# NUSTM/FacialMMT

Measured on AMD Instinct MI355X. Metric: utterances/sec T+A+V forward+bwd, 160-frame face seq, 1/2/4/8 GPU, higher is better.
Workload: dtype bf16; 1 GPU; configs[1]: T+A+V, RoBERTa-large (random init), 160-frame face seq (uint8 112x112 crops, fused pil-bicubic x2 + normalise), batch 4 utterances/GPU, bf16, fwd+bwd+clip+AdamW every step; global_batch=4, parallelism=dp1, hip_graphs=whole step: 2 graphs (fwd+bwd | clip+optimizer), text_encoder_concurrent_with_swin=True, swin_forward_pipelined_across_steps=False, text_encoder_parameters=bf16 with fp32 master weights in the optimizer

## Files before the change

facialmmt_amd/_lib.py:

```python
from __future__ import annotations

import ctypes as C
import os

_HERE = os.path.dirname(os.path.abspath(__file__))
LIB_PATH = os.path.join(_HERE, "libfmmt_hip.so")

F32, BF16 = 0, 1
GENERIC = 0x100
EPI_NONE, EPI_GELU, EPI_GELU_BWD, EPI_GELU_DG, EPI_MUL_AUX = 0, 1, 2, 3, 4
SAVE_DG = 0x200
BATCH_MAJOR = 0x400
RESIZE_PIL, RESIZE_CV2 = 0, 1

_p, _i, _f, _sz, _u64 = C.c_void_p, C.c_int, C.c_float, C.c_size_t, C.c_uint64

SIGNATURES = {
    "fmmt_version": (_i, []),
    "fmmt_linear_fwd": (_i, [_i, _i, _i, _i, _p, _i, _p, _i, _p, _p, _i, _p, _i, _p, _i, _p, _i, _p, _i, _p]),
    "fmmt_linear_splitk_workspace": (_sz, [_i, _i, _i]),
    "fmmt_linear_fwd_splitk": (_i, [_i, _i, _i, _i, _p, _i, _p, _i, _p, _p, _i, _p, _sz, _p]),
    "fmmt_linear_wgrad_workspace": (_sz, [_i, _i, _i, _i]),
    "fmmt_linear_wgrad": (_i, [_i, _i, _i, _i, _p, _i, _p, _i, _p, _p, _p, _i, _i, _p, _sz, _p]),
    "fmmt_linear_wgrad_partials": (_i, [_i, _i, _i, _i, _p, _i, _p, _i, _i, _p, _i, _i, _p, _sz, _p]),
    "fmmt_mlp_fwd": (_i, [_i, _i, _i, _p, _p, _p, _p, _p, _p, _p, _i, _p, _p, _p, _p]),
    "fmmt_mlp_ln_fwd": (_i, [_i, _i, _i, _p, _p, _p, _f, _p, _p, _p, _p, _p, _i, _p, _p, _p, _p, _p, _p, _p]),
    "fmmt_mlp_bwd_input": (_i, [_i, _i, _i, _p, _p, _p, _p, _p, _i, _p, _p, _p]),
    "fmmt_linear_ln_bwd_workspace": (_sz, [_i]),
    "fmmt_linear_ln_bwd": (_i, [_i, _i, _i, _i, _p, _p, _p, _p, _p, _p, _p, _p, _p, _p, _p, _sz, _p]),
    "fmmt_mlp_ln_bwd_input_workspace": (_sz, [_i]),
    "fmmt_mlp_ln_bwd_input": (_i, [_i, _i, _i, _p, _p, _p, _p, _p, _i, _p, _p, _p, _p, _p, _p, _p, _p, _p, _sz, _p]),
    "fmmt_linear_wgrad_finish": (_i, [_i, _i, _i, _i, _p, _p, _p, _sz, _p]),
    "fmmt_layernorm_fwd": (_i, [_i, _i, _i, _p, _p, _p, _f, _p, _p, _p, _i, _p]),
    "fmmt_layernorm_bwd_workspace": (_sz, [_i]),
    "fmmt_layernorm_bwd": (_i, [_i, _i, _i, _p, _p, _p, _p, _p, _p, _p, _p, _p, _i, _p, _sz, _p]),
    "fmmt_window_attn_fwd": (_i, [_i, _i, _i, _i, _i, _i, _i, _p, _p, _p, _p, _i, _i, _f, _p, _p, _p]),
    "fmmt_window_attn_bwd_workspace": (_sz, [_i]),
    "fmmt_window_attn_bwd": (_i, [_i, _i, _i, _i, _i, _i, _i, _p, _p, _p, _p, _p, _p, _p, _i, _i, _f, _p, _p, _p, _sz, _p]),
    "fmmt_window_block_fwd": (_i, [_i, _i, _i, _i, _i, _i, _i, _p, _p, _p, _f, _p, _p, _p, _p, _p, _p, _f, _p, _p, _p, _p, _p, _p, _p, _p]),
    "fmmt_window_block_fwd_ref": (_i, [_i, _i, _i, _i, _i, _i, _i, _p, _p, _p, _f, _p, _p, _p, _p, _p, _p, _f, _p, _p, _p, _p, _p, _p, _p, _p]),
    "fmmt_window_block_attn_bwd": (_i, [_i, _i, _i, _i, _i, _i, _i, _p, _p, _p, _p, _p, _p, _p, _p, _p, _f, _p, _p, _p, _p, _sz, _p]),
    "fmmt_window_block_attn_bwd_ref": (_i, [_i, _i, _i, _i, _i, _i, _i, _p, _p, _p, _p, _p, _p, _p, _p, _p, _f, _p, _p, _p, _p, _sz, _p]),
    "fmmt_linear_fwd_seg3": (_i, [_i, _i, _i, _i, _p, _i, _p, _p, _p, _i, _i, _p, _p, _p, _p, _i, _p]),
    "fmmt_select_frames_fwd": (_i, [_i, _i, _i, _i, _i, _i, _p, _p, _p, _p, _f, _p, _p, _p, _p]),
    "fmmt_select_frames_bwd": (_i, [_i, _i, _i, _i, _i, _i, _p, _p, _p, _p]),
    "fmmt_mha_fwd": (_i, [_i, _i, _i, _i, _i, _i, _p, _i, _p, _p, _i, _f, _p, _f, _u64, _p, _p, _i, _p, _p]),
    "fmmt_mha_bwd": (_i, [_i, _i, _i, _i, _i, _i, _p, _i, _p, _p, _i, _f, _p, _f, _u64, _p, _p, _p, _i, _p, _p, _i, _p, _p, _i, _p]),
    "fmmt_mha_avg_weights": (_i, [_i, _i, _i, _i, _i, _i, _p, _i, _p, _i, _f, _p, _f, _u64, _p, _p, _p, _p]),
    "fmmt_patch_im2col": (_i, [_i, _i, _p, _p, _p]),
    "fmmt_patch_col2im": (_i, [_i, _i, _p, _p, _p]),
    "fmmt_batchnorm1d_fwd": (_i, [_i, _i, _i, _p, _p, _p, _p, _p, _f, _f, _i, _p, _p, _p, _p]),
    "fmmt_batchnorm1d_bwd": (_i, [_i, _i, _i, _p, _p, _p, _p, _p, _i, _p, _p, _p, _p]),
    "fmmt_posemb_scale_fwd": (_i, [_i, _i, _i, _i, _p, _p, _f, _p, _p]),
    "fmmt_scale": (_i, [_i, _sz, _p, _f, _p, _p]),
    "fmmt_colsum": (_i, [_i, _i, _i, _i, _p, _i, _p, _p]),
    "fmmt_cast_batch": (_i, [_i, _i, _p, _p]),
    "fmmt_layernorm_bwd_bf16_workspace": (_sz, [_i, _i]),
    "fmmt_layernorm_bwd_bf16": (_i, [_i, _i, _f, _p, _p, _p, _p, _p, _p, _p, _sz, _p]),
    "fmmt_dropadd_ln_fwd": (_i, [_i, _i, _i, _f, _p, _p, _p, _p, _f, _u64, _p, _u64, _p, _p, _p]),
    "fmmt_dropadd_ln_bwd_workspace": (_sz, [_i, _i]),
    "fmmt_dropadd_ln_bwd": (_i, [_i, _i, _i, _f, _p, _p, _p, _f, _u64, _p, _u64, _p, _p, _p, _p, _p, _p, _sz, _p]),
    "fmmt_plm_dropadd_ln_fwd": (_i, [_i, _i, _f, _p, _p, _p, _p, _f, _u64, _p, _u64, _p, _p, _p]),
    "fmmt_embedding_bwd": (_i, [_i, _i, _i, _p, C.c_int64, _p, _p, _p]),
    "fmmt_plm_gelu_bwd_colsum_workspace": (_sz, [_i, _i]),
    "fmmt_plm_gelu_bwd_colsum": (_i, [_i, _i, _p, _p, _p, _p, _p, _sz, _p]),
    "fmmt_plm_dropadd_ln_bwd_workspace": (_sz, [_i, _i]),
    "fmmt_plm_dropadd_ln_bwd": (_i, [_i, _i, _f, _p, _p, _p, _f, _u64, _p, _u64, _p, _p, _p, _p, _p, _p, _sz, _p]),
    "fmmt_grad_handover": (_i, [_i, _i, _p, _p, _p, _p]),
    "fmmt_adamw_batch": (_i, [_i, _i, _p, _p, _p, _p, _f, _f, _f, _f, _f, _i, _p]),
    "fmmt_resize_table": (_i, [_i, _i, _i, _p, _p]),
    "fmmt_resize_band_rows": (_i, [_p, _i]),
    "fmmt_patch_embed_u8": (_i, [_i, _i, _i, _i, _p, _p, _p, _p, _p]),
    "fmmt_patch_embed_ln_fwd": (_i, [_i, _i, _i, _i, _p, _p, _p, _p, _p, _f, _p, _p, _p, _p, _p]),
    "fmmt_patch_embed_u8_ln_fwd": (_i, [_i, _i, _i, _i, _p, _p, _p, _p, _p, _p, _p, _f, _p, _p, _p, _p, _p, _p]),
    "fmmt_emotion_head_fwd": (_i, [_i, _i, _i, _i, _i, _p, _i, _p, _p, _p, _p, _p, _f, _p, _p, _p]),
    "fmmt_eval_accumulate": (_i, [_i, _i, _i, _p, _i, _p, _p, _p, _p, _p, _p, C.c_int64, C.c_int64, _p]),
}

FMMT_EINVAL, FMMT_EALIGN, FMMT_EWORKSPACE = -1, -2, -3
_ERR = {-1: "FMMT_EINVAL (bad shape / unsupported size)", -2: "FMMT_EALIGN (pointer or leading dimension not 16-byte aligned)",
        -3: "FMMT_EWORKSPACE (workspace too small)"}

_lib = None


class FmmtError(RuntimeError):
    pass


def load():
    global _lib
    if _lib is not None:
        return _lib
    if not os.path.exists(LIB_PATH):
# ... 25 lines not shown
```

facialmmt_amd/build.py:

```python
from __future__ import annotations

import glob
import os
import subprocess
import sys
from concurrent.futures import ThreadPoolExecutor

HERE = os.path.dirname(os.path.abspath(__file__))
CSRC = os.path.join(HERE, "csrc")
OUT = os.path.join(HERE, "libfmmt_hip.so")
SOURCES = ["gemm.hip", "layernorm.hip", "attn.hip", "wattn_mfma.hip", "wattn_bwd_ref.hip", "wblock.hip", "wblock_ref.hip", "mha_mfma.hip", "misc.hip", "preproc.hip", "mlp_fused.hip", "mlp_ref.hip", "patch_ln.hip", "lin_lnbwd.hip", "plm_fused.hip", "frame_filter.hip", "eval.hip"]
FLAGS = ["--offload-arch=gfx950", "-O3", "-std=c++17", "-fPIC", "-ffp-contract=fast"]


def _stale(target, deps):
    if not os.path.exists(target):
        return True
    t = os.path.getmtime(target)
    return any(os.path.getmtime(d) > t for d in deps)


def build(force: bool = False, verbose: bool = True, tag: str = "") -> str:
    hipcc = os.environ.get("HIPCC", "/opt/rocm/bin/hipcc")
    tag = tag or os.environ.get("FMMT_BUILD_TAG", "")
    csrc = os.environ.get("FMMT_CSRC_DIR", CSRC) if tag else CSRC
    headers = sorted(glob.glob(os.path.join(csrc, "*.h"))) + [os.path.join(csrc, "..", "..", "include", "fmmt.h")]
    objdir = os.path.join(HERE, "build_" + tag if tag else "build")
    out = os.path.join(HERE, f"libfmmt_hip_{tag}.so") if tag else OUT
    os.makedirs(objdir, exist_ok=True)
    jobs = []
    for s in SOURCES:
        src = os.path.join(csrc, s)
        obj = os.path.join(objdir, s.replace(".hip", ".o"))
        if force or _stale(obj, [src] + headers):
            jobs.append((src, obj))

    def cc(job):
        src, obj = job
        cmd = [hipcc] + FLAGS + os.environ.get("FMMT_CFLAGS", "").split() + ["-c", src, "-o", obj]
        if verbose:
            print(" ".join(cmd), flush=True)
        subprocess.run(cmd, check=True)

    with ThreadPoolExecutor(max_workers=4) as ex:
        list(ex.map(cc, jobs))
    objs = [os.path.join(objdir, s.replace(".hip", ".o")) for s in SOURCES]
    if force or jobs or _stale(out, objs):
        cmd = [hipcc, "--offload-arch=gfx950", "-shared", "-fPIC", "-o", out] + objs
        if verbose:
            print(" ".join(cmd), flush=True)
        subprocess.run(cmd, check=True)
    return out


if __name__ == "__main__":
    print(build(force="--force" in sys.argv))
```

facialmmt_amd/csrc/attn.hip:

```cpp
#include "fmmt_common.h"
#include "../../include/fmmt.h"
#include "wattn_args.h"
#include "mha_args.h"
#include <stdlib.h>

namespace {

constexpr int TOK = 49;
constexpr int WS = 7;
constexpr int HD = 32;
constexpr int KP = 36;
constexpr int BP = 50;
constexpr int WA_BWD_WAVES_PER_HEAD_MAX = 256;


template <typename T> __device__ __forceinline__ void load_row32(const T* p, float* r) {
    constexpr int VEC = Vec<T>::N;
#pragma unroll
    for (int c = 0; c < HD / VEC; ++c) {
        const Vec<T> v = ldvec<T>(p + c * VEC);
#pragma unroll
        for (int e = 0; e < VEC; ++e) r[c * VEC + e] = v.get(e);
    }
}
// ... 490 lines not shown
#pragma unroll 2
        for (int ii = 0; ii < MT; ++ii) {
            if (i0 + ii >= p.Lq) break;
            const float pij = __expf(ldot<D>(Qs + ii * P, kreg) + kb - Ls[ii]);
            const float ks = keep_scale(p, bh, i0 + ii, j);
            if constexpr (WHICH == 0) {
                laxpy<D>(acc, pij * ks, Gs + ii * P);
            } else {
                const float dP = ldot<D>(Gs + ii * P, vreg) * ks;
                laxpy<D>(acc, pij * (dP - Dl[ii]), Qs + ii * P);
            }
        }
    }
    if (active) {
        T* dst = reinterpret_cast<T*>(WHICH == 0 ? p.dv : p.dk);
        store_row<T, D>(dst + p.rk(j, b) * p.lddkv + h * D, acc);
    }
}

int mha_check(int dtype, int Lq, int Lk, int B, int E, int nH) {
    if (dtype != FMMT_BF16 && dtype != FMMT_F32) return FMMT_EINVAL;
    if (Lq <= 0 || Lk <= 0 || B <= 0 || nH <= 0 || E % nH) return FMMT_EINVAL;
    const int hd = E / nH;
    if (hd != 64 && hd != 32) return FMMT_EINVAL;
    return 0;
}


template <typename T>
__global__ __launch_bounds__(128) void mha_avg_weights_kernel(MhaArgs p, float* __restrict__ w) {
    extern __shared__ float qs[];
    const int i = blockIdx.x, b = blockIdx.y, hd = p.E / p.nH;
    const T* qg = reinterpret_cast<const T*>(p.q) + p.rq(i, b) * p.ldq;
    const T* kg = reinterpret_cast<const T*>(p.k);
    for (int c = threadIdx.x; c < p.E; c += 128) qs[c] = to_f32(qg[c]) * p.scale;
    __syncthreads();
    for (int j = threadIdx.x; j < p.Lk; j += 128) {
        const T* kr = kg + p.rk(j, b) * p.ldkv;
        const float kb = key_bias(p, b, j);
        float acc = 0.f;
        for (int h = 0; h < p.nH; ++h) {
            const int bh = b * p.nH + h;
            float s = 0.f;
            for (int d = 0; d < hd; ++d) s += qs[h * hd + d] * to_f32(kr[h * hd + d]);
            acc += __expf(s + kb - p.lse[(size_t)bh * p.Lq + i]) * keep_scale(p, bh, i, j);
        }
        w[((size_t)b * p.Lq + i) * p.Lk + j] = acc / (float)p.nH;
    }
}

}

extern "C" int fmmt_window_attn_fwd(int dtype, int n_img, int H, int W, int C, int num_heads, int shift,
                                    const void* qkv, const float* table, const int32_t* index,
                                    const float* mask, int nW_mask, int mask_is_shift, float scale,
                                    void* out, float* lse, void* stream) {
    if (int e = wa_check(dtype, n_img, H, W, C, num_heads, shift)) return e;
    if (mask && nW_mask <= 0) return FMMT_EINVAL;
    WaArgs a{};
    a.n_img = n_img; a.H = H; a.W = W; a.C = C; a.nH = num_heads; a.shift = shift; a.qkv = qkv; a.table = table;
    a.index = index; a.mask = mask; a.nW_mask = nW_mask; a.mask_is_shift = mask_is_shift; a.scale = scale; a.out = out; a.lse = lse;
    const int B_ = n_img * (H / WS) * (W / WS);
    a.groups_per_head = wa_groups_per_head(B_, num_heads, false, dtype == FMMT_BF16);
    a.xcd_grouped = wa_xcd_grouped(a.groups_per_head, dtype == FMMT_BF16);
    hipStream_t st = reinterpret_cast<hipStream_t>(stream);
    dim3 grid(num_heads * a.groups_per_head);
    if (dtype == FMMT_BF16) return fmmt_wattn_mfma_fwd_launch(a, (int)grid.x, st);
    hipLaunchKernelGGL(wattn_fwd_kernel<float>, grid, dim3(256), 0, st, a);
    FMMT_CHECK_LAUNCH();
    return 0;
}

static size_t wa_part_bytes(int num_heads) { return ((size_t)num_heads * (WA_BWD_WAVES_PER_HEAD_MAX + 1) * TOK * TOK * sizeof(float) + 255) / 256 * 256; }

extern "C" size_t fmmt_window_attn_bwd_workspace(int num_heads) {
    return wa_part_bytes(num_heads) + WA_SINK_BYTES;
}

extern "C" int fmmt_window_attn_bwd(int dtype, int n_img, int H, int W, int C, int num_heads, int shift,
                                    const void* qkv, const void* out, const void* dout, const float* lse,
                                    const float* table, const int32_t* index, const float* mask, int nW_mask,
                                    int mask_is_shift, float scale, void* dqkv, float* dtable,
                                    void* workspace, size_t workspace_bytes, void* stream) {
    const bool want_generic = (dtype & FMMT_GENERIC) != 0;
    dtype &= 0xff;
    if (int e = wa_check(dtype, n_img, H, W, C, num_heads, shift)) return e;
    if (mask && nW_mask <= 0) return FMMT_EINVAL;
    if (workspace_bytes < fmmt_window_attn_bwd_workspace(num_heads)) return FMMT_EWORKSPACE;
    const bool generic_ok = !mask || (mask_is_shift && shift > 0);
    if (want_generic && !generic_ok) return FMMT_EINVAL;
    const bool generic = want_generic || (dtype == FMMT_F32 && generic_ok);
    WaArgs a{};
    a.n_img = n_img; a.H = H; a.W = W; a.C = C; a.nH = num_heads; a.shift = shift; a.qkv = qkv; a.table = table;
    a.index = index; a.mask = mask; a.nW_mask = nW_mask; a.mask_is_shift = mask_is_shift; a.scale = scale; a.out = const_cast<void*>(out);
    a.lse = const_cast<float*>(lse); a.dout = dout; a.dqkv = dqkv; a.part = reinterpret_cast<float*>(workspace);
    a.sink = reinterpret_cast<char*>(workspace) + wa_part_bytes(num_heads);
    const int B_ = n_img * (H / WS) * (W / WS);
    a.groups_per_head = wa_groups_per_head(B_, num_heads, true, dtype == FMMT_BF16);
    a.xcd_grouped = wa_xcd_grouped(a.groups_per_head, dtype == FMMT_BF16);
    hipStream_t st = reinterpret_cast<hipStream_t>(stream);
    if (generic) {
        a.groups_per_head = fmmt_wattn_bwd_groups(B_, num_heads, 1);
        a.xcd_grouped = 0;
        if (int rc = fmmt_wattn_bwd_ref_launch(dtype, a, num_heads * a.groups_per_head, st)) return rc;
        return fmmt_wattn_dtable_finish(a.part, num_heads, a.groups_per_head, index, dtable, st);
    }
    dim3 grid(num_heads * a.groups_per_head);
    if (dtype == FMMT_BF16) {
        if (int rc = fmmt_wattn_mfma_bwd_launch(a, (int)grid.x, st)) return rc;
    } else {
        hipLaunchKernelGGL(wattn_bwd_kernel<float>, grid, dim3(256), 0, st, a);
        FMMT_CHECK_LAUNCH();
    }
    return fmmt_wattn_dtable_finish(a.part, num_heads, dtype == FMMT_BF16 ? a.groups_per_head : a.groups_per_head * 4, index, dtable, st);
}

static int wba_run(bool generic, int dtype, int n_img, int H, int W, int C, int num_heads, int shift,
                   const void* xn, const void* dy, const void* attn_out, const float* lse,
                   const void* wqkv, const float* bqkv, const void* wproj,
                   const float* table, const int32_t* index, float scale, const float* rowscale,
                   void* dqkv, float* dtable, void* workspace, size_t workspace_bytes, void* stream) {
    if (int e = wa_check(dtype, n_img, H, W, C, num_heads, shift)) return e;
    generic = generic || dtype == FMMT_F32;
    if ((dtype != FMMT_BF16 && dtype != FMMT_F32) || (C != 96 && C != 192) || (generic && C != 96)) return FMMT_EINVAL;
    if (!xn || !dy || !attn_out || !lse || !wqkv || !wproj || !table || !index || !dqkv || !dtable || !workspace) return FMMT_EINVAL;
    if (workspace_bytes < fmmt_window_attn_bwd_workspace(num_heads)) return FMMT_EWORKSPACE;
    WaArgs a{};
    a.n_img = n_img; a.H = H; a.W = W; a.C = C; a.nH = num_heads; a.shift = shift; a.table = table; a.index = index; a.scale = scale;
    a.mask_is_shift = shift > 0; a.out = const_cast<void*>(attn_out); a.lse = const_cast<float*>(lse); a.dout = dy; a.dqkv = dqkv;
    a.part = reinterpret_cast<float*>(workspace);
    a.sink = reinterpret_cast<char*>(workspace) + wa_part_bytes(num_heads);
    a.xn = xn; a.wqkv = wqkv; a.bqkv = bqkv; a.wproj = wproj; a.rowscale = rowscale;
    const int B_ = n_img * (H / WS) * (W / WS);
    hipStream_t st = reinterpret_cast<hipStream_t>(stream);
    if (generic) {
        a.groups_per_head = fmmt_wattn_bwd_groups(B_, num_heads, 1);
        if (int rc = fmmt_wattn_bwd_ref_launch(dtype, a, num_heads * a.groups_per_head, st)) return rc;
        return fmmt_wattn_dtable_finish(a.part, num_heads, a.groups_per_head, index, dtable, st);
    }
    a.groups_per_head = fmmt_wattn_bwd_groups(B_, num_heads, 4);
    a.xcd_grouped = wa_xcd_grouped(a.groups_per_head, true);
    if (int rc = fmmt_wattn_mfma_bwd_rc_launch(a, num_heads * a.groups_per_head, st)) return rc;
    return fmmt_wattn_dtable_finish(a.part, num_heads, a.groups_per_head, index, dtable, st);
}

extern "C" int fmmt_window_block_attn_bwd(int dtype, int n_img, int H, int W, int C, int num_heads, int shift,
                                          const void* xn, const void* dy, const void* attn_out, const float* lse,
                                          const void* wqkv, const float* bqkv, const void* wproj,
                                          const float* table, const int32_t* index, float scale, const float* rowscale,
                                          void* dqkv, float* dtable, void* workspace, size_t workspace_bytes, void* stream) {
    return wba_run(false, dtype, n_img, H, W, C, num_heads, shift, xn, dy, attn_out, lse, wqkv, bqkv, wproj, table, index, scale, rowscale,
                   dqkv, dtable, workspace, workspace_bytes, stream);
}

extern "C" int fmmt_window_block_attn_bwd_ref(int dtype, int n_img, int H, int W, int C, int num_heads, int shift,
                                              const void* xn, const void* dy, const void* attn_out, const float* lse,
                                              const void* wqkv, const float* bqkv, const void* wproj,
                                              const float* table, const int32_t* index, float scale, const float* rowscale,
                                              void* dqkv, float* dtable, void* workspace, size_t workspace_bytes, void* stream) {
    return wba_run(true, dtype, n_img, H, W, C, num_heads, shift, xn, dy, attn_out, lse, wqkv, bqkv, wproj, table, index, scale, rowscale,
                   dqkv, dtable, workspace, workspace_bytes, stream);
}

int fmmt_wattn_dtable_finish(float* part, int num_heads, int parts_per_head, const int32_t* index, float* dtable, hipStream_t st) {
    const int nt = (2 * WS - 1) * (2 * WS - 1) * num_heads;
    float* dense = part + (size_t)num_heads * WA_BWD_WAVES_PER_HEAD_MAX * TOK * TOK;
    const int nd = num_heads * TOK * TOK;
    hipLaunchKernelGGL(wattn_dense_kernel, dim3((nd + 63) / 64), dim3(256), 0, st, part, num_heads, parts_per_head, dense);
    FMMT_CHECK_LAUNCH();
    hipLaunchKernelGGL(wattn_dtable_kernel, dim3(nt), dim3(64), 0, st, dense, index, num_heads, dtable);
    FMMT_CHECK_LAUNCH();
    return 0;
}

int fmmt_wattn_bwd_groups(int B_, int num_heads, int windows_per_iteration) {
    int g = 256 / num_heads;
    const int maxg = (B_ + windows_per_iteration - 1) / windows_per_iteration;
    if (g > maxg) g = maxg;
    if (g > WA_BWD_WAVES_PER_HEAD_MAX) g = WA_BWD_WAVES_PER_HEAD_MAX;
    if (g >= 8) g &= ~7;
    return g < 1 ? 1 : g;
}

#define FMMT_MHA_DISPATCH(KERNEL, GRIDX)                                                             \
    do {                                                                                             \
        dim3 grid((GRIDX), B * num_heads);                                                           \
        const int hd = E / num_heads;                                                                \
        if (dtype == FMMT_BF16) {                                                                    \
// ... 67 lines not shown
```

facialmmt_amd/csrc/wattn_args.h:

```cpp
#pragma once
#include <hip/hip_runtime.h>
#include <stdint.h>

struct WaArgs {
    int n_img, H, W, C, nH, shift;
    const void* qkv;
    const float* table;
    const int32_t* index;
    const float* mask;
    int nW_mask;
    int mask_is_shift;
    float scale;
    void* out;
    float* lse;
    const void* dout;
    void* dqkv;
    float* part;
    int groups_per_head;
    int xcd_grouped;
    const void* xn;
    const void* wqkv;
    const float* bqkv;
    const void* wproj;
    const float* rowscale;
    void* sink;
};
constexpr size_t WA_SINK_BYTES = 16 * 1024;

int fmmt_wattn_mfma_fwd_launch(const WaArgs& a, int grid, hipStream_t st);
int fmmt_wattn_mfma_bwd_launch(const WaArgs& a, int grid, hipStream_t st);
int fmmt_wattn_mfma_bwd_rc_launch(const WaArgs& a, int grid, hipStream_t st);
int fmmt_wattn_bwd_ref_launch(int dtype, const WaArgs& a, int grid, hipStream_t st);

int fmmt_wattn_dtable_finish(float* part, int num_heads, int parts_per_head, const int32_t* index, float* dtable, hipStream_t st);
int fmmt_wattn_bwd_groups(int B_, int num_heads, int windows_per_iteration);
```

include/fmmt.h:

```cpp
#ifndef FMMT_H
#define FMMT_H
#include <stddef.h>
#include <stdint.h>

#ifdef __cplusplus
extern "C" {
#endif

#define FMMT_F32 0
#define FMMT_BF16 1
#define FMMT_GENERIC 0x100
#define FMMT_SAVE_DG 0x200
#define FMMT_BATCH_MAJOR 0x400

#define FMMT_EINVAL (-1)
#define FMMT_EALIGN (-2)
#define FMMT_EWORKSPACE (-3)

#define FMMT_EPI_GELU 1
#define FMMT_EPI_GELU_BWD 2
#define FMMT_EPI_GELU_DG 3
#define FMMT_EPI_MUL_AUX 4

int fmmt_version(void);

int fmmt_linear_fwd(int dtype, int M, int N, int K,
                    const void* x, int ldx, const void* w, int ldw, const float* bias,
                    void* y, int ldy, void* y_pre,
                    int epi, const void* aux, int ldaux,
                    const void* res, int ldres, const float* rowscale, int rows_per_scale,
                    void* stream);

int fmmt_linear_fwd_seg3(int dtype, int M, int N, int K, const void* x, int ldx, const void* w0, const void* w1, const void* w2, int ldw,
                         int seg_mode, const float* bias0, const float* bias1, const float* bias2, void* y, int ldy, void* stream);

size_t fmmt_linear_splitk_workspace(int M, int N, int K);
int fmmt_linear_fwd_splitk(int dtype, int M, int N, int K, const void* x, int ldx, const void* w, int ldw,
                           const float* bias, void* y, int ldy, void* workspace, size_t workspace_bytes,
                           void* stream);

size_t fmmt_linear_wgrad_workspace(int dtype, int M, int N, int K);
int fmmt_linear_wgrad(int dtype, int M, int N, int K,
                      const void* dy, int lddy, const void* x, int ldx,
                      float* dw, float* db, const float* rowscale, int rows_per_scale, int x_epi,
                      void* workspace, size_t workspace_bytes, void* stream);
int fmmt_linear_wgrad_partials(int dtype, int M, int N, int K,
                               const void* dy, int lddy, const void* x, int ldx, int want_bias,
                               const float* rowscale, int rows_per_scale, int x_epi,
                               void* workspace, size_t workspace_bytes, void* stream);
int fmmt_linear_wgrad_finish(int dtype, int M, int N, int K, float* dw, float* db,
                             const void* workspace, size_t workspace_bytes, void* stream);

int fmmt_mlp_fwd(int dtype, int M, int C, const void* x, const void* w1, const float* b1, const void* w2, const float* b2,
                 const void* res, const float* rowscale, int rows_per_scale, void* y, void* h_pre, void* h_act, void* stream);

int fmmt_mlp_ln_fwd(int dtype, int M, int C, const void* x, const float* ln_gamma, const float* ln_beta, float eps,
                    const void* w1, const float* b1, const void* w2, const float* b2, const float* rowscale, int rows_per_scale,
                    void* y, void* xn, float* mean, float* rstd, void* h_pre, void* h_act, void* stream);

int fmmt_mlp_bwd_input(int dtype, int M, int C, const void* dy, const void* h_pre, const void* w2t, const void* w1t,
                       const float* rowscale, int rows_per_scale, void* dh, void* dx, void* stream);

size_t fmmt_mlp_ln_bwd_input_workspace(int C);
int fmmt_mlp_ln_bwd_input(int dtype, int M, int C, const void* dy, const void* h_pre, const void* w2t, const void* w1t,
                          const float* rowscale, int rows_per_scale, const void* x, const float* mean, const float* rstd,
                          const float* ln_gamma, void* dh, void* dx, float* dgamma, float* dbeta, void* workspace,
                          size_t workspace_bytes, void* stream);

int fmmt_layernorm_fwd(int dtype, int M, int C, const void* x, const float* gamma, const float* beta,
                       float eps, void* y, float* mean, float* rstd, int merge_hw, void* stream);

size_t fmmt_layernorm_bwd_workspace(int C);
int fmmt_layernorm_bwd(int dtype, int M, int C, const void* dy, const void* x, const float* mean,
                       const float* rstd, const float* gamma, const void* add, void* dx,
                       float* dgamma, float* dbeta, int merge_hw,
                       void* workspace, size_t workspace_bytes, void* stream);

int fmmt_window_attn_fwd(int dtype, int n_img, int H, int W, int C, int num_heads, int shift,
                         const void* qkv, const float* table, const int32_t* index,
                         const float* mask, int nW_mask, int mask_is_shift, float scale,
                         void* out, float* lse, void* stream);

size_t fmmt_window_attn_bwd_workspace(int num_heads);
int fmmt_window_attn_bwd(int dtype, int n_img, int H, int W, int C, int num_heads, int shift,
                         const void* qkv, const void* out, const void* dout, const float* lse,
                         const float* table, const int32_t* index, const float* mask, int nW_mask,
                         int mask_is_shift, float scale, void* dqkv, float* dtable,
                         void* workspace, size_t workspace_bytes, void* stream);

int fmmt_window_block_fwd(int dtype, int n_img, int H, int W, int C, int num_heads, int shift,
                          const void* x, const float* ln_gamma, const float* ln_beta, float eps,
                          const void* wqkv, const float* bqkv, const void* wproj, const float* bproj,
                          const float* table, const int32_t* index, float scale, const float* rowscale,
                          void* y, void* xn, void* attn_out, float* mean, float* rstd, float* lse, void* stream);
int fmmt_window_block_fwd_ref(int dtype, int n_img, int H, int W, int C, int num_heads, int shift,
                              const void* x, const float* ln_gamma, const float* ln_beta, float eps,
// ... 109 lines not shown
```

Before: 74.11 utterances/s.

## Add 16-wave single-workgroup-per-CU window attention backward kernel

Adds a new bf16 window-attention backward kernel that runs 1024-thread workgroups. Each workgroup holds eight windows' K/Q/dO/V tiles in LDS with a swizzled layout and reads them back with transposed LDS loads. It computes dQ, dK, dV and the relative-position-bias gradient, and reduces d(bias) across waves in shared memory. It is enabled by default for C==768 and for shifted C==192 layers, with environment and flag overrides to force the old path. The aim is higher occupancy and more work per CU than the existing MFMA backward kernel. The cost is a large LDS footprint per workgroup and a serial cross-wave bias reduction.

```diff
diff --git a/facialmmt_amd/_lib.py b/facialmmt_amd/_lib.py
--- a/facialmmt_amd/_lib.py
+++ b/facialmmt_amd/_lib.py
@@ -10,6 +10,8 @@
 GENERIC = 0x100
 EPI_NONE, EPI_GELU, EPI_GELU_BWD, EPI_GELU_DG, EPI_MUL_AUX = 0, 1, 2, 3, 4
 SAVE_DG = 0x200
+WATTN_OCC = 0x1000
+WATTN_OLD = 0x800
 BATCH_MAJOR = 0x400
 RESIZE_PIL, RESIZE_CV2 = 0, 1
 
diff --git a/facialmmt_amd/build.py b/facialmmt_amd/build.py
--- a/facialmmt_amd/build.py
+++ b/facialmmt_amd/build.py
@@ -9,7 +9,7 @@
 HERE = os.path.dirname(os.path.abspath(__file__))
 CSRC = os.path.join(HERE, "csrc")
 OUT = os.path.join(HERE, "libfmmt_hip.so")
-SOURCES = ["gemm.hip", "layernorm.hip", "attn.hip", "wattn_mfma.hip", "wattn_bwd_ref.hip", "wblock.hip", "wblock_ref.hip", "mha_mfma.hip", "misc.hip", "preproc.hip", "mlp_fused.hip", "mlp_ref.hip", "patch_ln.hip", "lin_lnbwd.hip", "plm_fused.hip", "frame_filter.hip", "eval.hip"]
+SOURCES = ["gemm.hip", "layernorm.hip", "attn.hip", "wattn_mfma.hip", "wattn_bwd_occ.hip", "wattn_bwd_ref.hip", "wblock.hip", "wblock_ref.hip", "mha_mfma.hip", "misc.hip", "preproc.hip", "mlp_fused.hip", "mlp_ref.hip", "patch_ln.hip", "lin_lnbwd.hip", "plm_fused.hip", "frame_filter.hip", "eval.hip"]
 FLAGS = ["--offload-arch=gfx950", "-O3", "-std=c++17", "-fPIC", "-ffp-contract=fast"]
 
 
diff --git a/facialmmt_amd/csrc/attn.hip b/facialmmt_amd/csrc/attn.hip
--- a/facialmmt_amd/csrc/attn.hip
+++ b/facialmmt_amd/csrc/attn.hip
@@ -596,7 +596,7 @@
                                     const float* table, const int32_t* index, const float* mask, int nW_mask,
                                     int mask_is_shift, float scale, void* dqkv, float* dtable,
                                     void* workspace, size_t workspace_bytes, void* stream) {
-    const bool want_generic = (dtype & FMMT_GENERIC) != 0;
+    const bool want_generic = (dtype & FMMT_GENERIC) != 0, want_old = (dtype & FMMT_WATTN_OLD) != 0, want_occ = (dtype & FMMT_WATTN_OCC) != 0;
     dtype &= 0xff;
     if (int e = wa_check(dtype, n_img, H, W, C, num_heads, shift)) return e;
     if (mask && nW_mask <= 0) return FMMT_EINVAL;
@@ -618,6 +618,18 @@
         a.xcd_grouped = 0;
         if (int rc = fmmt_wattn_bwd_ref_launch(dtype, a, num_heads * a.groups_per_head, st)) return rc;
         return fmmt_wattn_dtable_finish(a.part, num_heads, a.groups_per_head, index, dtable, st);
+    }
+#ifndef FMMT_WATTN_OCC_DEFAULT
+#define FMMT_WATTN_OCC_DEFAULT 1
+#endif
+    static const int occ_on = fmmt_const("FMMT_WATTN_OCC", FMMT_WATTN_OCC_DEFAULT);
+    const bool occ_won = C == 768 || (C == 192 && mask && mask_is_shift);
+    if (dtype == FMMT_BF16 && !want_old && (want_occ || (occ_on && occ_won))) {
+        if (const int g = fmmt_wattn_bwd_occ_groups(a, B_, WA_BWD_WAVES_PER_HEAD_MAX)) {
+            a.groups_per_head = g;
+            if (int rc = fmmt_wattn_bwd_occ_launch(a, WA_BWD_WAVES_PER_HEAD_MAX, st)) return rc;
+            return fmmt_wattn_dtable_finish(a.part, num_heads, g, index, dtable, st);
+        }
     }
     dim3 grid(num_heads * a.groups_per_head);
     if (dtype == FMMT_BF16) {
diff --git a/facialmmt_amd/csrc/wattn_args.h b/facialmmt_amd/csrc/wattn_args.h
--- a/facialmmt_amd/csrc/wattn_args.h
+++ b/facialmmt_amd/csrc/wattn_args.h
@@ -30,6 +30,8 @@
 int fmmt_wattn_mfma_fwd_launch(const WaArgs& a, int grid, hipStream_t st);
 int fmmt_wattn_mfma_bwd_launch(const WaArgs& a, int grid, hipStream_t st);
 int fmmt_wattn_mfma_bwd_rc_launch(const WaArgs& a, int grid, hipStream_t st);
+int fmmt_wattn_bwd_occ_groups(const WaArgs& a, int B_, int max_groups);
+int fmmt_wattn_bwd_occ_launch(const WaArgs& a, int part_groups_max, hipStream_t st);
 int fmmt_wattn_bwd_ref_launch(int dtype, const WaArgs& a, int grid, hipStream_t st);
 
 int fmmt_wattn_dtable_finish(float* part, int num_heads, int parts_per_head, const int32_t* index, float* dtable, hipStream_t st);
diff --git a/facialmmt_amd/csrc/wattn_bwd_occ.hip b/facialmmt_amd/csrc/wattn_bwd_occ.hip
--- /dev/null
+++ b/facialmmt_amd/csrc/wattn_bwd_occ.hip
@@ -0,0 +1,323 @@
+#include "fmmt_common.h"
+#include "../../include/fmmt.h"
+#include "wattn_args.h"
+#include "wattn_geom.h"
+
+namespace {
+
+constexpr float OCC_LOG2E = 1.4426950408889634f;
+constexpr int OCC_NP = 8, OCC_NT = OCC_NP * 128;
+constexpr int OCC_TILE = 64 * HD;
+constexpr int OCC_TILES_B = 4 * OCC_NP * OCC_TILE * 2, OCC_STATS_B = 2 * OCC_NP * 64 * 4, OCC_BIAS_B = TOK * BPM * 4;
+constexpr int OCC_LDS = OCC_TILES_B + OCC_STATS_B + OCC_BIAS_B;
+static_assert(OCC_LDS <= 160 * 1024, "one workgroup per CU");
+static_assert((size_t)OCC_NT * 16 <= WA_SINK_BYTES, "every thread owns 16 bytes of the store sink");
+static_assert(3 * OCC_TILE * 2 >= TOK * TOK * 4, "the d(bias) reduction tile lies over the first three K tiles");
+
+__device__ __forceinline__ int occ_chunk(int c, int rq) { return c ^ ((4 - rq) & 3); }
+
+__device__ __forceinline__ int occ_row_off(int t, int li, int lg) { return (t * 16 + li) * HD + occ_chunk(lg, (li >> 2) & 3) * 8; }
+
+__device__ __forceinline__ bf16x8 occ_tr_frag(const bf16* tile, int rb, int lg, int dt, int li) {
+    const bf16* a0 = tile + (32 * rb + 4 * lg + (li >> 2)) * HD + occ_chunk(li & 3, lg) * 8 + dt * 4;
+    union { struct { s16x4 lo, hi; } s; bf16x8 v; } u;
+    u.s.lo = __builtin_amdgcn_ds_read_tr16_b64_v4i16((lds_s16x4*)(a0));
+    u.s.hi = __builtin_amdgcn_ds_read_tr16_b64_v4i16((lds_s16x4*)(a0 + 16 * HD));
+    return u.v;
+}
+
+struct OccSlot { int di, dj; bool valid; };
+__device__ __forceinline__ OccSlot occ_slot_of(int slot) {
+    OccSlot S;
+    S.valid = slot < TOK;
+    const int cs = S.valid ? slot : TOK - 1;
+    S.di = cs / WS;
+    S.dj = cs - S.di * WS;
+    return S;
+}
+
+template <int MM>
+__global__ __launch_bounds__(OCC_NT) void wattn_bwd_occ_kernel(WaArgs p) {
+    __shared__ __attribute__((aligned(16))) char smem_occ[OCC_LDS];
+    bf16* const tiles = reinterpret_cast<bf16*>(smem_occ);
+    float (*Ls)[64] = reinterpret_cast<float (*)[64]>(smem_occ + OCC_TILES_B);
+    float (*Dl)[64] = Ls + OCC_NP;
+    float* Bs = reinterpret_cast<float*>(smem_occ + OCC_TILES_B + OCC_STATS_B);
+    const int lane = threadIdx.x & 63, wave = __builtin_amdgcn_readfirstlane(threadIdx.x >> 6);
+    const int pair = wave >> 1, h = wave & 1;
+    const int li = lane & 15, lg = lane >> 4;
+#define OCC_LANE() int l_ = lane; asm volatile("" : "+v"(l_)); const int li = l_ & 15, lg = l_ >> 4
+
+    int head, grp;
+    {
+        const int b = blockIdx.x, gph = p.groups_per_head;
+        if (p.xcd_grouped) {
+            const int u = (b >> 4) * 8 + (b & 7);
+            if (u >= (p.nH >> 1) * gph) return;
+            const int hp = u / gph;
+            head = hp * 2 + ((b >> 3) & 1);
+            grp = u - hp * gph;
+        } else {
+            head = b / gph;
+            grp = b - head * gph;
+        }
+    }
+    const int nW = (p.H / WS) * (p.W / WS), B_ = p.n_img * nW;
+    const int stride = p.groups_per_head * OCC_NP;
+    const bf16* __restrict__ qkv = reinterpret_cast<const bf16*>(p.qkv);
+    const bf16* __restrict__ og = reinterpret_cast<const bf16*>(p.out);
+    const bf16* __restrict__ dog = reinterpret_cast<const bf16*>(p.dout);
+    bf16* __restrict__ dqkv = reinterpret_cast<bf16*>(p.dqkv);
+    const LaneGeom G = lane_geom(li, lg, p.shift);
+    bf16 *kt_ = tiles + pair * OCC_TILE, *qt_ = kt_ + OCC_NP * OCC_TILE, *gt_ = qt_ + OCC_NP * OCC_TILE, *vt_ = gt_ + OCC_NP * OCC_TILE;
+    bf16* const sink_w = reinterpret_cast<bf16*>(p.sink) + wave * 64 * 8;
+
+    for (int t = threadIdx.x; t < TOK * BPM; t += OCC_NT) {
+        const int q = t / BPM, k = t - q * BPM;
+        Bs[t] = k < TOK ? p.table[p.index[q * TOK + k] * p.nH + head] * OCC_LOG2E : NEG_BIG;
+    }
+    const float sc2 = p.scale * OCC_LOG2E;
+    f32x4 dbias[2][4];
+#pragma unroll
+    for (int a = 0; a < 2; ++a)
+#pragma unroll
+        for (int b = 0; b < 4; ++b) dbias[a][b] = f32x4{0.f, 0.f, 0.f, 0.f};
+
+    const int iters = (B_ + stride - 1) / stride;
+    for (int it = 0; it < iters; ++it) {
+        const int b_raw = it * stride + grp * OCC_NP + pair;
+        const bool wactive = b_raw < B_;
+        const int b_ = wactive ? b_raw : B_ - 1;
+        const WinPos P = win_pos(p, b_);
+        int tok[2];
+        bf16x8 qf[2], kf[2], gf[2], vv[2], of[2];
+        float ls[2], dl[2];
+        {
+        OCC_LANE();
+#pragma unroll
+        for (int a = 0; a < 2; ++a) {
+            const OccSlot own = occ_slot_of((2 * h + a) * 16 + li);
+            tok[a] = (int)tok_of(p, P, own.di, own.dj);
+            const bf16* row = qkv + (size_t)tok[a] * 3 * p.C + head * HD + lg * 8;
+            qf[a] = ld_frag(row);
+            kf[a] = ld_frag(row + p.C);
+            vv[a] = ld_frag(row + 2 * p.C);
+            gf[a] = ld_frag(dog + (size_t)tok[a] * p.C + head * HD + lg * 8);
+            of[a] = ld_frag(og + (size_t)tok[a] * p.C + head * HD + lg * 8);
+            const int slot = (2 * h + a) * 16 + li;
+            ls[a] = p.lse[((size_t)b_ * p.nH + head) * TOK + (slot < TOK ? slot : TOK - 1)];
+        }
+        }
+        __syncthreads();
+        {
+        OCC_LANE();
+#pragma unroll
+        for (int a = 0; a < 2; ++a) {
+            const int slot = (2 * h + a) * 16 + li;
+            const bool valid = slot < TOK;
+            float d = 0.f;
+#pragma unroll
+            for (int e = 0; e < 8; ++e) d += (float)gf[a][e] * (float)of[a][e];
+            dl[a] = xor_sum(d);
+            ls[a] = valid ? ls[a] * OCC_LOG2E : 1.0e30f;
+            const int off = occ_row_off(2 * h + a, li, lg);
+            kf[a] = valid ? kf[a] : zero_frag();
+            qf[a] = valid ? qf[a] : zero_frag();
+            gf[a] = valid ? gf[a] : zero_frag();
+            vv[a] = valid ? vv[a] : zero_frag();
+            *reinterpret_cast<bf16x8*>(kt_ + off) = kf[a];
+            *reinterpret_cast<bf16x8*>(qt_ + off) = qf[a];
+            *reinterpret_cast<bf16x8*>(gt_ + off) = gf[a];
+            *reinterpret_cast<bf16x8*>(vt_ + off) = vv[a];
+            if (lg == 0) {
+                Ls[pair][slot] = ls[a];
+                Dl[pair][slot] = dl[a];
+            }
+        }
+        }
+        __syncthreads();
+
+#pragma unroll
+        for (int a = 0; a < 2; ++a) {
+            OCC_LANE();
+            const int qt = 2 * h + a;
+            const int q = qt * 16 + li;
+            const float* brow = Bs + (q < TOK ? q : TOK - 1) * BPM + lg * 4;
+            float ds[8];
+            bf16x8 dpk[2];
+            const unsigned mb = (MM == 1) ? std_mask_bits(G, P, qt) : 0u;
+            const bf16x8 qfa = ld_frag(qt_ + occ_row_off(qt, li, lg)), gfa = ld_frag(gt_ + occ_row_off(qt, li, lg));
+            const float lsa = Ls[pair][q], dla = Dl[pair][q];
+#pragma unroll
+            for (int ktp = 0; ktp < 4; ++ktp) {
+                const int kt = ktp;
+                const bf16x8 kfk = ld_frag(kt_ + occ_row_off(kt, li, lg));
+                const f32x4 sa = __builtin_amdgcn_mfma_f32_16x16x32_bf16(kfk, qfa, f32x4{0.f, 0.f, 0.f, 0.f}, 0, 0, 0);
+                const bf16x8 vfk = ld_frag(vt_ + occ_row_off(kt, li, lg));
+                const f32x4 dp = __builtin_amdgcn_mfma_f32_16x16x32_bf16(vfk, gfa, f32x4{0.f, 0.f, 0.f, 0.f}, 0, 0, 0);
+                const f32x4 b = *reinterpret_cast<const f32x4*>(brow + kt * 16);
+                const unsigned mbk = mb >> (kt * 4);
+#pragma unroll
+                for (int r = 0; r < 4; ++r) {
+                    const float s = sa[r] * sc2 + b[r];
+                    float pij = __builtin_amdgcn_exp2f(s - lsa);
+                    if constexpr (MM == 1) pij = ((mbk >> r) & 1u) ? 0.0f : pij;
+                    const float d = pij * (dp[r] - dla);
+                    ds[(ktp & 1) * 4 + r] = d;
+                    if (wactive) dbias[a][ktp][r] += d;
+                }
+                if (ktp & 1) {
+                    dpk[ktp >> 1] = pack8(&ds[0], &ds[4]);
+                    __builtin_amdgcn_sched_barrier(0);
+                }
+            }
+            const bf16x8 d0 = dpk[0], d1 = dpk[1];
+            __builtin_amdgcn_sched_barrier(0);
+            bf16x8 kT[2][2];
+#pragma unroll
+            for (int ks = 0; ks < 2; ++ks)
+#pragma unroll
+                for (int dt = 0; dt < 2; ++dt) kT[ks][dt] = occ_tr_frag(kt_, ks, lg, dt, li);
+            f32x4 a0 = {0.f, 0.f, 0.f, 0.f}, a1 = {0.f, 0.f, 0.f, 0.f};
+            a0 = __builtin_amdgcn_mfma_f32_16x16x32_bf16(kT[0][0], d0, a0, 0, 0, 0);
+            a0 = __builtin_amdgcn_mfma_f32_16x16x32_bf16(kT[1][0], d1, a0, 0, 0, 0);
+            a1 = __builtin_amdgcn_mfma_f32_16x16x32_bf16(kT[0][1], d0, a1, 0, 0, 0);
+            a1 = __builtin_amdgcn_mfma_f32_16x16x32_bf16(kT[1][1], d1, a1, 0, 0, 0);
+            {
+                bf16x8 ob;
+#pragma unroll
+                for (int r = 0; r < 4; ++r) { ob[r] = (bf16)(a0[r] * p.scale); ob[4 + r] = (bf16)(a1[r] * p.scale); }
+                *reinterpret_cast<bf16x8*>((wactive && q < TOK) ? dqkv + (size_t)tok[a] * 3 * p.C + head * HD + lg * 8 : sink_w + l_ * 8) = ob;
+            }
+            __builtin_amdgcn_sched_barrier(0);
+        }
+
+#pragma unroll
+        for (int a = 0; a < 2; ++a) {
+            OCC_LANE();
+            const int kt = 2 * h + a;
+            const int key = kt * 16 + li;
+            float pp[8], ds[8];
+            bf16x8 ppk[2], dpk[2];
+            const unsigned mb = (MM == 1) ? std_mask_bits(G, P, kt) : 0u;
+            const bf16x8 kfa = ld_frag(kt_ + occ_row_off(kt, li, lg)), vfa = ld_frag(vt_ + occ_row_off(kt, li, lg));
+            const float* bcol = Bs + key;
+#pragma unroll
+            for (int qtp = 0; qtp < 4; ++qtp) {
+                const int qt = qtp;
+                const bf16x8 qfq = ld_frag(qt_ + occ_row_off(qt, li, lg));
+                const bf16x8 gfq = ld_frag(gt_ + occ_row_off(qt, li, lg));
+                const f32x4 sa = __builtin_amdgcn_mfma_f32_16x16x32_bf16(qfq, kfa, f32x4{0.f, 0.f, 0.f, 0.f}, 0, 0, 0);
+                const f32x4 dp = __builtin_amdgcn_mfma_f32_16x16x32_bf16(gfq, vfa, f32x4{0.f, 0.f, 0.f, 0.f}, 0, 0, 0);
+                const f32x4 lq = *reinterpret_cast<const f32x4*>(&Ls[pair][qt * 16 + lg * 4]);
+                const f32x4 dq = *reinterpret_cast<const f32x4*>(&Dl[pair][qt * 16 + lg * 4]);
+                const unsigned mbq = mb >> (qt * 4);
+#pragma unroll
+                for (int r = 0; r < 4; ++r) {
+                    const int q = qt * 16 + lg * 4 + r;
+                    const float s = sa[r] * sc2 + bcol[(q < TOK ? q : TOK - 1) * BPM];
+                    float pij = __builtin_amdgcn_exp2f(s - lq[r]);
+                    if constexpr (MM == 1) pij = ((mbq >> r) & 1u) ? 0.0f : pij;
+                    pp[(qtp & 1) * 4 + r] = pij;
+                    ds[(qtp & 1) * 4 + r] = pij * (dp[r] - dq[r]);
+                }
+                if (qtp & 1) {
+                    ppk[qtp >> 1] = pack8(&pp[0], &pp[4]);
+                    dpk[qtp >> 1] = pack8(&ds[0], &ds[4]);
+                }
+                __builtin_amdgcn_sched_barrier(0);
+            }
+            const bf16x8 p0 = ppk[0], p1 = ppk[1], d0 = dpk[0], d1 = dpk[1];
+            __builtin_amdgcn_sched_barrier(0);
+            f32x4 v0 = {0.f, 0.f, 0.f, 0.f}, v1 = {0.f, 0.f, 0.f, 0.f}, k0 = {0.f, 0.f, 0.f, 0.f}, k1 = {0.f, 0.f, 0.f, 0.f};
+            {
+                bf16x8 gT[2][2];
+#pragma unroll
+                for (int qs = 0; qs < 2; ++qs)
+#pragma unroll
+                    for (int dt = 0; dt < 2; ++dt) gT[qs][dt] = occ_tr_frag(gt_, qs, lg, dt, li);
+                v0 = __builtin_amdgcn_mfma_f32_16x16x32_bf16(gT[0][0], p0, v0, 0, 0, 0);
+                v0 = __builtin_amdgcn_mfma_f32_16x16x32_bf16(gT[1][0], p1, v0, 0, 0, 0);
+                v1 = __builtin_amdgcn_mfma_f32_16x16x32_bf16(gT[0][1], p0, v1, 0, 0, 0);
+                v1 = __builtin_amdgcn_mfma_f32_16x16x32_bf16(gT[1][1], p1, v1, 0, 0, 0);
+            }
+            {
+                bf16x8 qT[2][2];
+#pragma unroll
+                for (int qs = 0; qs < 2; ++qs)
+#pragma unroll
+                    for (int dt = 0; dt < 2; ++dt) qT[qs][dt] = occ_tr_frag(qt_, qs, lg, dt, li);
+                k0 = __builtin_amdgcn_mfma_f32_16x16x32_bf16(qT[0][0], d0, k0, 0, 0, 0);
+                k0 = __builtin_amdgcn_mfma_f32_16x16x32_bf16(qT[1][0], d1, k0, 0, 0, 0);
+                k1 = __builtin_amdgcn_mfma_f32_16x16x32_bf16(qT[0][1], d0, k1, 0, 0, 0);
+                k1 = __builtin_amdgcn_mfma_f32_16x16x32_bf16(qT[1][1], d1, k1, 0, 0, 0);
+            }
+            {
+                bf16x8 kb, vb;
+#pragma unroll
+                for (int r = 0; r < 4; ++r) {
+                    kb[r] = (bf16)(k0[r] * p.scale); kb[4 + r] = (bf16)(k1[r] * p.scale);
+                    vb[r] = (bf16)v0[r]; vb[4 + r] = (bf16)v1[r];
+                }
+                const bool live = wactive && key < TOK;
+                bf16* const sinkp = sink_w + l_ * 8;
+                bf16* dst = dqkv + (size_t)tok[a] * 3 * p.C + head * HD + lg * 8;
+                *reinterpret_cast<bf16x8*>(live ? dst + p.C : sinkp) = kb;
+                *reinterpret_cast<bf16x8*>(live ? dst + 2 * p.C : sinkp) = vb;
+            }
+            __builtin_amdgcn_sched_barrier(0);
+        }
+    }
+    float* acc = reinterpret_cast<float*>(tiles);
+    for (int w = 0; w < 2 * OCC_NP; ++w) {
+        __syncthreads();
+        if (wave == w) {
+#pragma unroll
+            for (int a = 0; a < 2; ++a) {
+                const int q = (2 * h + a) * 16 + li;
+                if (q >= TOK) continue;
+#pragma unroll
+                for (int ktp = 0; ktp < 4; ++ktp)
+#pragma unroll
+                    for (int r = 0; r < 4; ++r) {
+                        const int key = ktp * 16 + lg * 4 + r;
+                        if (key < TOK) {
+                            const float v = dbias[a][ktp][r];
+                            acc[q * TOK + key] = (w < 2) ? v : acc[q * TOK + key] + v;
+                        }
+                    }
+            }
+        }
+    }
+    __syncthreads();
+    float* part = p.part + ((size_t)head * p.groups_per_head + grp) * TOK * TOK;
+    for (int t = threadIdx.x; t < TOK * TOK; t += OCC_NT) part[t] = acc[t];
+}
+
+template <int MM>
+int occ_launch(const WaArgs& a, int grid, hipStream_t st) {
+    hipLaunchKernelGGL((wattn_bwd_occ_kernel<MM>), dim3(grid), dim3(OCC_NT), 0, st, a);
+    FMMT_CHECK_LAUNCH();
+    return 0;
+}
+
+}
+
+int fmmt_wattn_bwd_occ_groups(const WaArgs& a, int B_, int max_groups) {
+    const int mm = !a.mask ? 0 : (a.mask_is_shift ? 1 : 2);
+    if (mm == 2 || a.nH > 256) return 0;
+    int g = 256 / a.nH;
+    const int maxg = (B_ + OCC_NP - 1) / OCC_NP;
+    if (g > maxg) g = maxg;
+    if (g > max_groups) g = max_groups;
+    return g < 1 ? 1 : g;
+}
+
+int fmmt_wattn_bwd_occ_launch(const WaArgs& a_, int part_groups_max, hipStream_t st) {
+    WaArgs a = a_;
+    const int mm = !a.mask ? 0 : (a.mask_is_shift ? 1 : 2);
+    if (mm == 2 || a.groups_per_head < 1 || a.groups_per_head > part_groups_max || !a.sink || !a.part) return FMMT_EINVAL;
+    a.xcd_grouped = (a.nH % 2 == 0) ? 1 : 0;
+    const int grid = a.xcd_grouped ? (((a.nH / 2) * a.groups_per_head + 7) / 8) * 16 : a.nH * a.groups_per_head;
+    return mm == 0 ? occ_launch<0>(a, grid, st) : occ_launch<1>(a, grid, st);
+}
diff --git a/include/fmmt.h b/include/fmmt.h
--- a/include/fmmt.h
+++ b/include/fmmt.h
@@ -12,6 +12,8 @@
 #define FMMT_GENERIC 0x100
 #define FMMT_SAVE_DG 0x200
 #define FMMT_BATCH_MAJOR 0x400
+#define FMMT_WATTN_OLD 0x800
+#define FMMT_WATTN_OCC 0x1000
 
 #define FMMT_EINVAL (-1)
 #define FMMT_EALIGN (-2)
```

Measured after the change: 73.78 utterances/s. No clear change (-0.5%).
